# h33p/ofps

Measured on AMD Instinct MI355X. Metric: Mvectors/s, 1080p 16x16 blocks +-16 full-search SAD, higher is better.
Workload: dtype u8

## Files before the change

ofps_amd/csrc/sad.hip:

```cpp
#include "common.hpp"

#include <cstdlib>
#include <utility>

namespace {

constexpr int kWavesPerWG = 4;

constexpr int pick_stride(int min_s, int k, int ng) {
    for (int s = min_s; s < min_s + 64; ++s)
        if ((k * s) % 32 == ng % 32) return s;
    return min_s | 1;
}

template <int B, int R, int K>
struct SadCfg {
    static_assert(B % 4 == 0 && R % 4 == 0, "tile origin must stay dword aligned");
    static_assert(B * B * 255 <= 65535, "packed u16 SAD accumulators would overflow");
    static constexpr int NCAND = 2 * R + 1;
    static constexpr int NG = (NCAND + 3) / 4;
    static constexpr int NC = (NCAND + K - 1) / K;
    static constexpr int T = NG * NC;
    static constexpr int PASSES = (T + 63) / 64;
    static constexpr int BW = B / 4;
    static constexpr int TILE_H = B + 2 * R;
    static constexpr int TILE_ROWS = NC * K + B - 1;
    static constexpr int TILE_WD = (kWavesPerWG * B + 2 * R) / 4;
    static constexpr int MAXCOL = (kWavesPerWG - 1) * BW + (NG - 1) + BW;
    static constexpr int MIN_S = (MAXCOL + 1 > TILE_WD) ? MAXCOL + 1 : TILE_WD;
    static constexpr int S = pick_stride(MIN_S, K, NG);
    static constexpr int LDS_DWORDS = TILE_ROWS * S;
};

__device__ __forceinline__ unsigned long long shfl_xor_u64(unsigned long long v, int mask) {
    unsigned lo = (unsigned)v, hi = (unsigned)(v >> 32);
    lo = __shfl_xor(lo, mask, 64);
    hi = __shfl_xor(hi, mask, 64);
    return ((unsigned long long)hi << 32) | lo;
}

struct __attribute__((packed, aligned(4))) U64A4 { unsigned long long v; };

struct SadParams {
    const uint8_t* prev_base;
    const uint8_t* cur_base;
    size_t prev_pitch, cur_pitch;
    int W, H, stride;
    int nbx, nby;
    float nx, ny;
    float4* out_entries;
    int* out_best;
    unsigned long long div_spp, div_spr;
};
inline unsigned long long div_magic48(unsigned d) { return ((1ull << 48) + d - 1) / d; }
__device__ __forceinline__ unsigned div48(unsigned n, unsigned long long m) { return (unsigned)(((unsigned long long)n * m) >> 48); }

__device__ __forceinline__ void write_block_result(const SadParams& p, int pair, int bx, int by, int B, int R,
                                                   unsigned long long key) {
    const int sad = (int)(key >> 48);
    const int dy = (int)((key >> 8) & 0xFF) - R;
    const int dx = (int)(key & 0xFF) - R;
    const size_t k = ((size_t)pair * p.nby + by) * p.nbx + bx;
    const float cx = (float)(bx * B + B / 2 + dx), cy = (float)(by * B + B / 2 + dy);
    float4 e;
    e.x = cx * p.nx;
    e.y = cy * p.ny;
    e.z = ((float)dx / 1.0f) * (-p.nx);
    e.w = ((float)dy / 1.0f) * (-p.ny);
    p.out_entries[k] = e;
    if (p.out_best) {
        p.out_best[3 * k + 0] = dx;
        p.out_best[3 * k + 1] = dy;
        p.out_best[3 * k + 2] = sad;
    }
}

template <int B, int R, int K>
__global__ __launch_bounds__(256) void sad_qsad_kernel(const SadParams p) {
    using C = SadCfg<B, R, K>;
    __shared__ uint32_t tile[C::LDS_DWORDS];

    const int pair = blockIdx.z;
    const uint8_t* __restrict__ prev = p.prev_base + (size_t)pair * p.prev_pitch;
    const uint8_t* __restrict__ cur = p.cur_base + (size_t)pair * p.cur_pitch;
    const int by = blockIdx.y;
    const int bx0 = blockIdx.x * kWavesPerWG;
    const int tid = threadIdx.x;

    const int wave = __builtin_amdgcn_readfirstlane(tid >> 6);
    const int lane = tid & 63;
    const int bx = bx0 + wave;
    const int x0 = bx * B, y0 = by * B;

    uint32_t c[B][C::BW];
    {
        const int bxc = bx < p.nbx ? bx : p.nbx - 1;
        const uint32_t* __restrict__ cp = reinterpret_cast<const uint32_t*>(cur + (size_t)y0 * p.stride + bxc * B);
        const int sdw = p.stride >> 2;
#pragma unroll
        for (int y = 0; y < B; ++y)
#pragma unroll
            for (int q = 0; q < C::BW; ++q) c[y][q] = cp[y * sdw + q];
    }

    {
        const int tx0 = bx0 * B - R, ty0 = by * B - R;
        for (int idx = tid; idx < C::TILE_H * C::TILE_WD; idx += 256) {
            const int row = idx / C::TILE_WD, col = idx - row * C::TILE_WD;
            const int gx = tx0 + 4 * col, gy = ty0 + row;
            if (gy >= 0 && gy < p.H && gx >= 0 && gx < p.W)
                tile[row * C::S + col] = *reinterpret_cast<const uint32_t*>(prev + (size_t)gy * p.stride + gx);
        }
    }
    __syncthreads();
    if (bx >= p.nbx) return;

    unsigned long long best = ~0ull;
#pragma unroll 1
    for (int pass = 0; pass < C::PASSES; ++pass) {
        const int t = pass * 64 + lane;
        const bool active = t < C::T;
        const int tc = active ? t : 0;
        const int chunk = tc / C::NG, g = tc - chunk * C::NG;
        const int dx0 = -R + 4 * g, dy0 = -R + K * chunk;

        unsigned long long acc[K];
#pragma unroll
        for (int i = 0; i < K; ++i) acc[i] = 0;

        const uint32_t* trow = tile + (K * chunk) * C::S + wave * C::BW + g;
#pragma unroll
        for (int rr = 0; rr < B + K - 1; ++rr) {
            unsigned long long win[C::BW];
#pragma unroll
            for (int q = 0; q < C::BW; ++q) win[q] = reinterpret_cast<const U64A4*>(trow + rr * C::S + q)->v;
#pragma unroll
            for (int i = 0; i < K; ++i) {
                const int y = rr - i;
                if (y >= 0 && y < B) {
#pragma unroll
                    for (int q = 0; q < C::BW; ++q) acc[i] = __builtin_amdgcn_qsad_pk_u16_u8(win[q], c[y][q], acc[i]);
                }
            }
        }
        __builtin_amdgcn_sched_group_barrier(0x100, C::BW, 0);
#pragma unroll
        for (int rr = 0; rr < B + K - 1; ++rr) {
            __builtin_amdgcn_sched_group_barrier(0x100, C::BW, 0);
            __builtin_amdgcn_sched_group_barrier(0x002, K * C::BW, 0);
        }

#pragma unroll
        for (int i = 0; i < K; ++i) asm volatile("" : "+v"(acc[i]));

        uint32_t bkey = 0xFFFFFFFFu;
        int bci = 0;
#pragma unroll
        for (int i = 0; i < K; ++i) {
            const int dy = dy0 + i;
            const int vy = (int)active & (int)(dy <= R) & (int)(y0 + dy >= 0) & (int)(y0 + dy + B <= p.H);
#pragma unroll
            for (int j = 0; j < 4; ++j) {
                const int dx = dx0 + j;
                const int v = vy & (int)(dx <= R) & (int)(x0 + dx >= 0) & (int)(x0 + dx + B <= p.W);
                const uint32_t d2inv = (uint32_t)(dx * dx + dy * dy) | (uint32_t)(v - 1);
                const uint32_t half = (j < 2) ? (uint32_t)acc[i] : (uint32_t)(acc[i] >> 32);
                const uint32_t key = ((j & 1) ? (half & 0xFFFF0000u) : (half << 16)) | d2inv;
                const bool lt = key < bkey;
                bkey = lt ? key : bkey;
                bci = lt ? (i * 4 + j) : bci;
            }
        }
        if (bkey != 0xFFFFFFFFu) {
            const int bi = bci >> 2, bj = bci & 3;
            const unsigned long long k64 =
                ((unsigned long long)bkey << 32) | (uint32_t)(((dy0 + bi + R) << 8) | (dx0 + bj + R));
            best = k64 < best ? k64 : best;
        }
    }

#pragma unroll
    for (int m = 32; m >= 1; m >>= 1) {
        const unsigned long long o = shfl_xor_u64(best, m);
        best = o < best ? o : best;
    }
    if (lane == 0) write_block_result(p, pair, bx, by, B, R, best);
}

template <int B, int R>
struct StripCfg {
    static_assert(B % 4 == 0 && R % 4 == 0, "tile origin and the dx = +R column must stay dword aligned");
    static_assert(B * B * 255 <= 65535, "packed u16 SAD accumulators would overflow");
    static constexpr int NCAND = 2 * R + 1;
    static constexpr int NGA = (2 * R) / 4;
    static constexpr int pow2_ceil(int v) { int p = 1; while (p < v) p <<= 1; return p; }
    static constexpr int NG = pow2_ceil(NGA);
    static_assert(NGA >= 1 && NG <= 64, "search range too wide for one wave per strip");
    static constexpr int NB = 64 / NG;
    static constexpr int BW = B / 4;
    static constexpr int TILE_H = B + 2 * R;
    static constexpr int KE = (NCAND + NG - 1) / NG;
    static constexpr int EDGE_COL = (2 * R) / 4;
    static constexpr int GRAN = ((NB * B) % 16 == 0 && R % 16 == 0) ? 16 : (((NB * B) % 8 == 0 && R % 8 == 0) ? 8 : 4);
    static constexpr int GDW = GRAN / 4;
    static constexpr int TILE_WG = (NB * B + 2 * R + GRAN - 1) / GRAN;
    static constexpr int MAXCOL = (NB - 1) * BW + (NG - 1) + BW;
    static constexpr int SW = ((MAXCOL + 1 > TILE_WG * GDW ? MAXCOL + 1 : TILE_WG * GDW) + 3) / 4 * 4;
    static_assert((NB - 1) * BW + EDGE_COL + BW <= SW, "edge column must lie inside a window row");
    static constexpr int TILE_ROWS = TILE_H > NG * KE + B - 1 ? TILE_H : NG * KE + B - 1;
    static constexpr int TILE_DWORDS = TILE_ROWS * SW;
    static_assert(2 * R * R < 65536, "lane key holds d2 in 16 bits");
    static constexpr int SPLIT = (NCAND + 32) / 33;
    static constexpr int NP = (NCAND + SPLIT - 1) / SPLIT;
    static constexpr int MIN_WAVES = (2 * NP + B * BW + 40 <= 168) ? 3 : 2;
    static constexpr bool COMPACT_KEY = ((2 * R * R) << 6) + NCAND < 65536 && NCAND <= 64;
    static constexpr bool RANK_KEY = !COMPACT_KEY && ((2 * R * R) << 3) + 7 < 65536;
    static constexpr int KSHIFT = COMPACT_KEY ? 6 : (RANK_KEY ? 3 : 0);
};

template <int B, int R>
struct StripWalk {
    static constexpr int ROWS_PER_BASE = (255 - StripCfg<B, R>::BW) / StripCfg<B, R>::SW + 1;
};

template <int B, int R, int I0, int RR>
__device__ __forceinline__ void strip_row(unsigned long long (&acc)[StripCfg<B, R>::NP], const uint32_t (&c)[B][B / 4],
                                          const uint32_t* lds, uint32_t& base) {
    using C = StripCfg<B, R>;
    constexpr int G = StripWalk<B, R>::ROWS_PER_BASE;
    if constexpr (RR > 0 && RR % G == 0) {
        base += G * C::SW;
        asm volatile("" : "+v"(base));
    }
    unsigned long long win[C::BW];
#pragma unroll
    for (int q = 0; q < C::BW; ++q) win[q] = reinterpret_cast<const U64A4*>(lds + base + (RR % G) * C::SW + q)->v;
#pragma unroll
    for (int ii = 0; ii < C::NP; ++ii) {
        const int y = RR - ii;
        if (I0 + ii < C::NCAND && y >= 0 && y < B) {
#pragma unroll
            for (int q = 0; q < C::BW; ++q) acc[ii] = __builtin_amdgcn_qsad_pk_u16_u8(win[q], c[y][q], acc[ii]);
        }
    }
}

template <int B, int R, int I0, int... RR>
__device__ __forceinline__ void strip_rows(unsigned long long (&acc)[StripCfg<B, R>::NP], const uint32_t (&c)[B][B / 4],
                                           const uint32_t* lds, uint32_t tile_off, std::integer_sequence<int, RR...>) {
    uint32_t base = tile_off + I0 * StripCfg<B, R>::SW;
    asm volatile("" : "+v"(base));
    (strip_row<B, R, I0, RR>(acc, c, lds, base), ...);
}

#ifndef OFPS_SAD_COLKEYS
#define OFPS_SAD_COLKEYS 2
#endif
constexpr int kSadColKeys = OFPS_SAD_COLKEYS;
constexpr int kColSlotDwords = kSadColKeys == 2 ? 4 * 64 : 0;

template <int B, int R, int I0>
__device__ __forceinline__ void strip_pass(const uint32_t (&c)[B][B / 4], const uint32_t* lds, uint32_t tile_off,
                                           const uint32_t (&colk)[4], const uint32_t (&colk_pos)[4], int y0, int H, uint32_t& bkey, int& bi,
                                           uint32_t (&colmin)[4], uint32_t* amin) {
    using C = StripCfg<B, R>;
    unsigned long long acc[C::NP];
#pragma unroll
    for (int ii = 0; ii < C::NP; ++ii) acc[ii] = 0;
    constexpr int ROWS = ((I0 + C::NP < C::NCAND ? C::NP : C::NCAND - I0) + B - 1);
    strip_rows<B, R, I0>(acc, c, lds, tile_off, std::make_integer_sequence<int, ROWS>{});
#pragma unroll
    for (int ii = 0; ii < C::NP; ++ii) asm volatile("" : "+v"(acc[ii]));
    if constexpr (kSadColKeys != 0 && (C::RANK_KEY || C::COMPACT_KEY)) {
        auto low_of = [&](int ii) -> uint32_t {
            const int i = I0 + ii, dy = -R + i;
            const bool ok = i < C::NCAND && y0 + dy >= 0 && y0 + dy + B <= H;
            return ok ? (uint32_t)(C::RANK_KEY ? ((dy * dy) << 1 | (dy > 0 ? 1 : 0)) : ((dy * dy) << 6 | i)) : 0xFFFFFFFFu;
        };
        uint32_t hmask = 0xFFFF0000u;
        asm volatile("" : "+v"(hmask));
        auto keys_of = [&](int ii, uint32_t low, uint32_t (&k)[4]) {
            const uint32_t lo = (uint32_t)acc[ii], hi = (uint32_t)(acc[ii] >> 32);
            k[0] = (lo << 16) | low; k[1] = (lo & hmask) | low; k[2] = (hi << 16) | low; k[3] = (hi & hmask) | low;
        };
        if constexpr (kSadColKeys == 1) {
#pragma unroll
            for (int ii = 0; ii < C::NP; ii += 2) {
                if (I0 + ii >= C::NCAND) break;
                uint32_t ka[4], kb[4];
                keys_of(ii, low_of(ii), ka);
                if (ii + 1 < C::NP && I0 + ii + 1 < C::NCAND) {
                    keys_of(ii + 1, low_of(ii + 1), kb);
#pragma unroll
                    for (int j = 0; j < 4; ++j)
                        asm("v_min3_u32 %0, %1, %2, %3" : "=v"(colmin[j]) : "v"(colmin[j]), "v"(ka[j]), "v"(kb[j]));
                } else {
#pragma unroll
                    for (int j = 0; j < 4; ++j) colmin[j] = min(colmin[j], ka[j]);
                }
            }
        } else {
#pragma unroll
            for (int ii = 0; ii < C::NP; ++ii) {
                if (I0 + ii >= C::NCAND) break;
                uint32_t k[4];
                keys_of(ii, low_of(ii), k);
#pragma unroll
                for (int j = 0; j < 4; ++j) __hip_atomic_fetch_min(amin + 64 * j, k[j], __ATOMIC_RELAXED, __HIP_MEMORY_SCOPE_WAVEFRONT);
            }
        }
        return;
    }
#pragma unroll
    for (int ii = 0; ii < C::NP; ++ii) {
        const int i = I0 + ii;
        const int dy = -R + i;
        if (i < C::NCAND && y0 + dy >= 0 && y0 + dy + B <= H) {
            const uint32_t lo = (uint32_t)acc[ii], hi = (uint32_t)(acc[ii] >> 32);
            const uint32_t (&ck)[4] = (C::RANK_KEY && dy > 0) ? colk_pos : colk;
            const uint32_t k0 = (lo << 16) | ck[0];
            const uint32_t k1 = (lo & 0xFFFF0000u) | ck[1];
            const uint32_t k2 = (hi << 16) | ck[2];
            const uint32_t k3 = (hi & 0xFFFF0000u) | ck[3];
            if constexpr (C::RANK_KEY) {
                bkey = min(bkey, __builtin_elementwise_add_sat(min(min(k0, k1), min(k2, k3)), (uint32_t)((dy * dy) << 3)));
            } else if constexpr (C::COMPACT_KEY) {
                const uint32_t m = __builtin_elementwise_add_sat(min(min(k0, k1), min(k2, k3)), (uint32_t)((dy * dy) << 6 | i));
                bkey = min(bkey, m);
            } else {
                const uint32_t m = __builtin_elementwise_add_sat(min(min(k0, k1), min(k2, k3)), (uint32_t)(dy * dy));
                const bool lt = m < bkey;
                bkey = lt ? m : bkey;
                bi = lt ? i : bi;
            }
        }
    }
}

template <int B, int R, int... S>
__device__ __forceinline__ void strip_passes(const uint32_t (&c)[B][B / 4], const uint32_t* lds, uint32_t tile_off,
                                             const uint32_t (&colk)[4], const uint32_t (&colk_pos)[4], int y0, int H, uint32_t& bkey, int& bi,
                                             uint32_t (&colmin)[4], uint32_t* amin, std::integer_sequence<int, S...>) {
    (strip_pass<B, R, S * StripCfg<B, R>::NP>(c, lds, tile_off, colk, colk_pos, y0, H, bkey, bi, colmin, amin), ...);
}

constexpr int kStripWaves = 4;

template <int B, int R>
__device__ __forceinline__ void strip_body(const SadParams& p, int strips_per_row, int strip, uint32_t* tiles, int wave, int lane) {
    using C = StripCfg<B, R>;
    const int strips_per_pair = strips_per_row * p.nby;
    const int pair = (int)div48((unsigned)strip, p.div_spp);
    const int rem = strip - pair * strips_per_pair;
    const int by = (int)div48((unsigned)rem, p.div_spr);
    const int bx0 = (rem - by * strips_per_row) * C::NB;

    const uint8_t* __restrict__ prev = p.prev_base + (size_t)pair * p.prev_pitch;
    const uint8_t* __restrict__ cur = p.cur_base + (size_t)pair * p.cur_pitch;
    uint32_t* tile = tiles + wave * C::TILE_DWORDS;

    const int b = lane / C::NG;
    const int g = lane % C::NG;
    const int bx = bx0 + b;
    const bool blk_on = bx < p.nbx;
    const int y0 = by * B;

    uint32_t c[B][C::BW];
    {
        const int bxc = blk_on ? bx : p.nbx - 1;
        const uint8_t* cp = cur + (size_t)y0 * p.stride + bxc * B;
#pragma unroll
        for (int y = 0; y < B; ++y) {
            if constexpr (C::BW % 4 == 0) {
#pragma unroll
                for (int q4 = 0; q4 < C::BW; q4 += 4) {
                    const uint4 v = *reinterpret_cast<const uint4*>(cp + (size_t)y * p.stride + 4 * q4);
                    c[y][q4 + 0] = v.x; c[y][q4 + 1] = v.y; c[y][q4 + 2] = v.z; c[y][q4 + 3] = v.w;
                }
            } else {
#pragma unroll
                for (int q2 = 0; q2 < C::BW; q2 += 2) {
                    const uint2 v = *reinterpret_cast<const uint2*>(cp + (size_t)y * p.stride + 4 * q2);
                    c[y][q2 + 0] = v.x; c[y][q2 + 1] = v.y;
                }
            }
        }
    }

    {
        constexpr int LR = 64 / C::TILE_WG;
        constexpr int STEPS = (C::TILE_H + LR - 1) / LR;
        const int tx0 = bx0 * B - R, ty0 = y0 - R;
        const int sr = lane / C::TILE_WG, sc = lane - sr * C::TILE_WG;
        const int gx = tx0 + C::GRAN * sc;
        const bool lane_on = sr < LR && gx >= 0 && gx < p.W;
        const uint8_t* src = prev + (ptrdiff_t)(ty0 + sr) * p.stride + gx;
        uint32_t* dst = tile + sr * C::SW + C::GDW * sc;
#pragma unroll
        for (int it = 0; it < STEPS; ++it) {
            const int row = sr + it * LR;
            const bool row_in_tile = (it + 1) * LR <= C::TILE_H || row < C::TILE_H;
            if (lane_on && row_in_tile && (unsigned)(ty0 + row) < (unsigned)p.H) {
                const uint8_t* sp = src + (ptrdiff_t)(it * LR) * p.stride;
                uint32_t* dp = dst + it * LR * C::SW;
                if constexpr (C::GRAN == 16) *reinterpret_cast<uint4*>(dp) = *reinterpret_cast<const uint4*>(sp);
                else if constexpr (C::GRAN == 8) *reinterpret_cast<uint2*>(dp) = *reinterpret_cast<const uint2*>(sp);
                else *dp = *reinterpret_cast<const uint32_t*>(sp);
            }
        }
    }
    __builtin_amdgcn_fence(__ATOMIC_RELEASE, "wavefront");
    __builtin_amdgcn_wave_barrier();
    __builtin_amdgcn_fence(__ATOMIC_ACQUIRE, "wavefront");

    const int dx0 = -R + 4 * g;
    uint32_t colk[4], colk_pos[4];
#pragma unroll
    for (int j = 0; j < 4; ++j) {
        const int dx = dx0 + j;
        const int x = bx * B + dx;
        const bool v = blk_on && g < C::NGA && x >= 0 && x + B <= p.W;
        const uint32_t rank = dx0 < 0 ? 3u - j : (uint32_t)j;
        colk[j] = v ? ((uint32_t)(dx * dx) << C::KSHIFT) | (C::RANK_KEY ? rank : 0u) : 0xFFFFFFFFu;
        colk_pos[j] = v ? ((uint32_t)(dx * dx) << C::KSHIFT) | (7u - rank) : 0xFFFFFFFFu;
    }
    uint32_t bkey = 0xFFFFFFFFu;
    int bi = 0;
    uint32_t colmin[4] = {0xFFFFFFFFu, 0xFFFFFFFFu, 0xFFFFFFFFu, 0xFFFFFFFFu};
    uint32_t* amin = nullptr;
    if constexpr (kSadColKeys == 2 && (C::RANK_KEY || C::COMPACT_KEY)) {
        amin = tiles + kStripWaves * C::TILE_DWORDS + wave * kColSlotDwords + lane;
#pragma unroll
        for (int j = 0; j < 4; ++j) amin[64 * j] = 0xFFFFFFFFu;
    }
    strip_passes<B, R>(c, tiles, (uint32_t)(wave * C::TILE_DWORDS + b * C::BW + g), colk, colk_pos, y0, p.H, bkey, bi, colmin, amin,
                       std::make_integer_sequence<int, C::SPLIT>{});
    if constexpr (kSadColKeys != 0 && (C::RANK_KEY || C::COMPACT_KEY)) {
#pragma unroll
        for (int j = 0; j < 4; ++j) {
            uint32_t kc;
            if constexpr (kSadColKeys == 2) kc = __hip_atomic_load(amin + 64 * j, __ATOMIC_RELAXED, __HIP_MEMORY_SCOPE_WAVEFRONT);
            else kc = colmin[j];
            uint32_t lk;
            if constexpr (C::RANK_KEY) {
                const uint32_t x = (((kc & 0xFFFEu) << 2) + colk[j]) ^ ((kc & 1u) * 7u);
                lk = (kc & 0xFFFF0000u) | x;
            } else {
                lk = (kc & 0xFFFF0000u) | ((kc & 0xFFFFu) + colk[j]);
            }
            lk = (colk[j] == 0xFFFFFFFFu || kc == 0xFFFFFFFFu) ? 0xFFFFFFFFu : lk;
            bkey = min(bkey, lk);
        }
    }
    unsigned long long best = ~0ull;
    if (bkey != 0xFFFFFFFFu) {
        const uint32_t d2 = (bkey & 0xFFFFu) >> C::KSHIFT;
        int dx = dx0, dy;
        if constexpr (C::RANK_KEY) {
            const int code = (int)(bkey & 7u);
            const bool neg = code < 4;
            const int rank = neg ? code : 7 - code;
            dx = dx0 + (dx0 < 0 ? 3 - rank : rank);
            const int ady = (int)(__builtin_sqrtf((float)((int)d2 - dx * dx)) + 0.5f);
            dy = neg ? -ady : ady;
        } else {
            if constexpr (C::COMPACT_KEY) bi = (int)(bkey & 63u);
            dy = -R + bi;
            const int dxsq = (int)d2 - dy * dy;
#pragma unroll
            for (int j = 1; j < 4; ++j) dx = ((dx0 + j) * (dx0 + j) == dxsq) ? dx0 + j : dx;
        }
        best = ((unsigned long long)((bkey & 0xFFFF0000u) | d2) << 32) | (unsigned long long)(uint32_t)(((dy + R) << 8) | (dx + R));
    }
    uint32_t eacc[C::KE];
#pragma unroll
    for (int i = 0; i < C::KE; ++i) eacc[i] = 0;
    {
        const uint32_t* ecol = tile + b * C::BW + C::EDGE_COL;
        const int erow0 = g * C::KE;
        uint32_t nxt[C::BW];
#pragma unroll
        for (int q = 0; q < C::BW; ++q) nxt[q] = ecol[erow0 * C::SW + q];
#pragma unroll
        for (int rr = 0; rr < B + C::KE - 1; ++rr) {
            uint32_t ref[C::BW];
#pragma unroll
            for (int q = 0; q < C::BW; ++q) ref[q] = nxt[q];
            if (rr + 1 < B + C::KE - 1) {
                const int row = erow0 + rr + 1;
#pragma unroll
                for (int q = 0; q < C::BW; ++q) nxt[q] = ecol[row * C::SW + q];
            }
#pragma unroll
            for (int i = 0; i < C::KE; ++i) {
                const int y = rr - i;
                if (y >= 0 && y < B) {
#pragma unroll
                    for (int q = 0; q < C::BW; ++q) eacc[i] = __builtin_amdgcn_sad_u8(ref[q], c[y][q], eacc[i]);
                }
            }
            asm volatile("" : "+v"(eacc[0]) : : "memory");
        }
    }

    {
        const bool xok = blk_on && bx * B + R + B <= p.W;
#pragma unroll
        for (int i = 0; i < C::KE; ++i) {
            const int dy = -R + g * C::KE + i;
            const bool v = xok && dy <= R && y0 + dy >= 0 && y0 + dy + B <= p.H;
            const unsigned long long k64 =
                ((unsigned long long)((eacc[i] << 16) | (uint32_t)(R * R + dy * dy)) << 32) |
                (unsigned long long)(uint32_t)(((dy + R) << 8) | (2 * R));
            best = (v && k64 < best) ? k64 : best;
        }
    }
#pragma unroll
    for (int m = 1; m < C::NG; m <<= 1) {
        const unsigned long long o = shfl_xor_u64(best, m);
        best = o < best ? o : best;
    }
    if (blk_on && g == 0) {
        const int sad = (int)(best >> 48);
        const int dy = (int)((best >> 8) & 0xFF) - R, dx = (int)(best & 0xFF) - R;
        const size_t k = ((size_t)pair * p.nby + by) * p.nbx + bx;
        float4 e;
        e.x = (float)(bx * B + B / 2 + dx) * p.nx;
        e.y = (float)(y0 + B / 2 + dy) * p.ny;
        e.z = ((float)dx / 1.0f) * (-p.nx);
        e.w = ((float)dy / 1.0f) * (-p.ny);
        p.out_entries[k] = e;
        if (p.out_best) {
            p.out_best[3 * k + 0] = dx;
            p.out_best[3 * k + 1] = dy;
            p.out_best[3 * k + 2] = sad;
        }
    }
}

template <int B, int R>
__global__ __launch_bounds__(64 * kStripWaves, (StripCfg<B, R>::MIN_WAVES)) void sad_strip_kernel(const SadParams p, int strips_per_row,
                                                                      int total_strips) {
    using C = StripCfg<B, R>;
    __shared__ __attribute__((aligned(16))) uint32_t tiles[kStripWaves * (C::TILE_DWORDS + kColSlotDwords)];
    const int wave = __builtin_amdgcn_readfirstlane(threadIdx.x >> 6);
    const int lane = threadIdx.x & 63;
    const int per_xcd = gridDim.x / 8;
    const int lwg = (int)(blockIdx.x % 8) * per_xcd + (int)(blockIdx.x / 8);
    const int strip = lwg * kStripWaves + wave;
    if (strip >= total_strips) return;
    strip_body<B, R>(p, strips_per_row, strip, tiles, wave, lane);
}

template <int B, int R>
__global__ __launch_bounds__(64 * kStripWaves, (StripCfg<B, R>::MIN_WAVES)) void sad_strip_list_kernel(const SadParams p, int strips_per_row,
                                                                           const uint32_t* __restrict__ strip_list) {
    using C = StripCfg<B, R>;
    __shared__ __attribute__((aligned(16))) uint32_t tiles[kStripWaves * (C::TILE_DWORDS + kColSlotDwords)];
    const int wave = __builtin_amdgcn_readfirstlane(threadIdx.x >> 6);
    const int lane = threadIdx.x & 63;
    const int count = (int)strip_list[0];
#pragma unroll 1
    for (int k = (int)blockIdx.x * kStripWaves + wave; k < count; k += (int)gridDim.x * kStripWaves)
        strip_body<B, R>(p, strips_per_row, (int)strip_list[1 + k], tiles, wave, lane);
}

struct PdeCfg {
    static constexpr int B = 16, R = 16, STEP = 4, PR = B / STEP;
    using C = StripCfg<B, R>;
    static constexpr int CUR_DW = B * C::NB * C::BW;
    static constexpr int CAP = 512;
    static constexpr int WAVE_DW = C::TILE_DWORDS + 4 + CUR_DW + CAP + 2 * C::NB;
    static constexpr int OFF_CUR = C::TILE_DWORDS + 4, OFF_LIST = OFF_CUR + CUR_DW, OFF_BEST = OFF_LIST + CAP;
    static_assert(OFF_BEST % 2 == 0, "64-bit keys must be 8-byte aligned");
};

template <int RR>
__device__ __forceinline__ void pde_row(unsigned long long (&acc)[PdeCfg::C::NP], const uint32_t (&c)[PdeCfg::PR][PdeCfg::C::BW],
                                        const uint32_t* lds, uint32_t& base) {
    using C = PdeCfg::C;
    constexpr int B = PdeCfg::B, R = PdeCfg::R, STEP = PdeCfg::STEP;
    constexpr int G = StripWalk<B, R>::ROWS_PER_BASE;
    if constexpr (RR > 0 && RR % G == 0) {
        base += G * C::SW;
        asm volatile("" : "+v"(base));
    }
    unsigned long long win[C::BW];
#pragma unroll
    for (int q = 0; q < C::BW; ++q) win[q] = reinterpret_cast<const U64A4*>(lds + base + (RR % G) * C::SW + q)->v;
#pragma unroll
    for (int ii = 0; ii < C::NP; ++ii) {
        const int y = RR - ii;
        if (ii < C::NCAND && y >= 0 && y < B && y % STEP == 0) {
#pragma unroll
            for (int q = 0; q < C::BW; ++q) acc[ii] = __builtin_amdgcn_qsad_pk_u16_u8(win[q], c[y / STEP][q], acc[ii]);
        }
    }
}
template <int... RR>
__device__ __forceinline__ void pde_rows(unsigned long long (&acc)[PdeCfg::C::NP], const uint32_t (&c)[PdeCfg::PR][PdeCfg::C::BW],
                                         const uint32_t* lds, uint32_t tile_off, std::integer_sequence<int, RR...>) {
    uint32_t base = tile_off;
    asm volatile("" : "+v"(base));
    (pde_row<RR>(acc, c, lds, base), ...);
}

__device__ __forceinline__ uint32_t pde_two_rows(const uint32_t* tile, const uint32_t* curl, int bb, int dyi, int dxi, int r8) {
    using C = PdeCfg::C;
    const int sh = dxi & 3;
    uint32_t s = 0;
#pragma unroll
    for (int k = 0; k < 2; ++k) {
        const int y = 2 * r8 + k;
        const uint32_t* rp = tile + (dyi + y) * C::SW + bb * C::BW + (dxi >> 2);
        const uint32_t* cp = curl + y * (C::NB * C::BW) + bb * C::BW;
        uint32_t d[C::BW + 1];
#pragma unroll
        for (int q = 0; q <= C::BW; ++q) d[q] = rp[q];
#pragma unroll
        for (int q = 0; q < C::BW; ++q) s = __builtin_amdgcn_sad_u8(__builtin_amdgcn_alignbyte(d[q + 1], d[q], sh), cp[q], s);
    }
    return s;
}

__global__ __launch_bounds__(64 * kStripWaves, 3) void sad_pde_kernel(const SadParams p, int strips_per_row, int total_strips,
                                                                       uint32_t* __restrict__ strip_list) {
    using P = PdeCfg;
    using C = P::C;
    constexpr int B = P::B, R = P::R;
    __shared__ __attribute__((aligned(16))) uint32_t lds[kStripWaves * P::WAVE_DW];

    const int wave = __builtin_amdgcn_readfirstlane(threadIdx.x >> 6);
    const int lane = threadIdx.x & 63;
    const int per_xcd = gridDim.x / 8;
    const int lwg = (int)(blockIdx.x % 8) * per_xcd + (int)(blockIdx.x / 8);
    const int strip = lwg * kStripWaves + wave;
    if (strip >= total_strips) return;
    const int strips_per_pair = strips_per_row * p.nby;
    const int pair = strip / strips_per_pair;
    const int rem = strip - pair * strips_per_pair;
    const int by = rem / strips_per_row;
    const int bx0 = (rem - by * strips_per_row) * C::NB;
    const uint8_t* __restrict__ prev = p.prev_base + (size_t)pair * p.prev_pitch;
    const uint8_t* __restrict__ cur = p.cur_base + (size_t)pair * p.cur_pitch;
    uint32_t* tile = lds + wave * P::WAVE_DW;
    uint32_t* curl = tile + P::OFF_CUR;
    uint32_t* list = tile + P::OFF_LIST;
    unsigned long long* bestk = reinterpret_cast<unsigned long long*>(tile + P::OFF_BEST);

    const int b = lane / C::NG, g = lane % C::NG;
    const int bx = bx0 + b;
    const bool blk_on = bx < p.nbx;
    const int y0 = by * B;

    {
        const int tx0 = bx0 * B - R, ty0 = y0 - R;
        for (int idx = lane; idx < C::TILE_H * C::TILE_WG; idx += 64) {
            const int row = idx / C::TILE_WG, col = idx - row * C::TILE_WG;
            const int gx = tx0 + 16 * col, gy = ty0 + row;
            if (gy >= 0 && gy < p.H && gx >= 0 && gx < p.W)
                *reinterpret_cast<uint4*>(tile + row * C::SW + 4 * col) = *reinterpret_cast<const uint4*>(prev + (size_t)gy * p.stride + gx);
        }
#pragma unroll
        for (int k = 0; k < 2; ++k) {
            const int idx = lane + 64 * k, row = idx / C::NB, blk = idx % C::NB;
            const int bxc = min(bx0 + blk, p.nbx - 1);
            *reinterpret_cast<uint4*>(curl + row * (C::NB * C::BW) + blk * C::BW) =
                *reinterpret_cast<const uint4*>(cur + (size_t)(y0 + row) * p.stride + bxc * B);
        }
    }
    __builtin_amdgcn_fence(__ATOMIC_RELEASE, "wavefront");
    __builtin_amdgcn_wave_barrier();
    __builtin_amdgcn_fence(__ATOMIC_ACQUIRE, "wavefront");

    uint32_t c4[P::PR][C::BW];
#pragma unroll
    for (int r = 0; r < P::PR; ++r)
#pragma unroll
        for (int q = 0; q < C::BW; ++q) c4[r][q] = curl[(P::STEP * r) * (C::NB * C::BW) + b * C::BW + q];
    unsigned long long acc[C::NP];
#pragma unroll
    for (int ii = 0; ii < C::NP; ++ii) acc[ii] = 0;
    pde_rows(acc, c4, lds, (uint32_t)(wave * P::WAVE_DW + b * C::BW + g), std::make_integer_sequence<int, C::NCAND + B - 1>{});
#pragma unroll
    for (int ii = 0; ii < C::NP; ++ii) asm volatile("" : "+v"(acc[ii]));

    const int dx0 = -R + 4 * g;
    bool colv[4];
    uint32_t colk[4];
#pragma unroll
    for (int j = 0; j < 4; ++j) {
        const int x = bx * B + dx0 + j;
        colv[j] = blk_on && x >= 0 && x + B <= p.W;
        colk[j] = colv[j] ? (uint32_t)((dx0 + j) * (dx0 + j)) << C::KSHIFT : 0xFFFFFFFFu;
    }
    static_assert(C::COMPACT_KEY && C::SPLIT == 1, "written for the +-16 geometry");
    uint32_t bkey = 0xFFFFFFFFu;
#pragma unroll
    for (int i = 0; i < C::NCAND; ++i) {
        const int dy = -R + i;
        if (y0 + dy >= 0 && y0 + dy + B <= p.H) {
            const uint32_t lo = (uint32_t)acc[i], hi = (uint32_t)(acc[i] >> 32);
            const uint32_t k0 = (lo << 16) | colk[0], k1 = (lo & 0xFFFF0000u) | colk[1];
            const uint32_t k2 = (hi << 16) | colk[2], k3 = (hi & 0xFFFF0000u) | colk[3];
            bkey = min(bkey, __builtin_elementwise_add_sat(min(min(k0, k1), min(k2, k3)), (uint32_t)((dy * dy) << 6 | i)));
        }
    }
    unsigned long long pbest = ~0ull;
    if (bkey != 0xFFFFFFFFu) {
        const int bi = (int)(bkey & 63u), dy = -R + bi;
        const uint32_t d2 = (bkey & 0xFFFFu) >> C::KSHIFT;
        const int dxsq = (int)d2 - dy * dy;
        int dx = dx0;
#pragma unroll
        for (int j = 1; j < 4; ++j) dx = ((dx0 + j) * (dx0 + j) == dxsq) ? dx0 + j : dx;
        pbest = ((unsigned long long)((bkey & 0xFFFF0000u) | d2) << 32) | (unsigned long long)(uint32_t)(((dy + R) << 8) | (dx + R));
    }
    uint32_t eacc[C::KE];
    const bool xok = blk_on && bx * B + R + B <= p.W;
    {
        const uint32_t* ecol = tile + b * C::BW + C::EDGE_COL;
#pragma unroll
        for (int i = 0; i < C::KE; ++i) {
            const int dyi = min(g * C::KE + i, C::NCAND - 1);
            uint32_t sacc = 0;
#pragma unroll
            for (int r = 0; r < P::PR; ++r)
#pragma unroll
                for (int q = 0; q < C::BW; ++q) sacc = __builtin_amdgcn_sad_u8(ecol[(dyi + P::STEP * r) * C::SW + q], c4[r][q], sacc);
            eacc[i] = sacc;
            const int dy = -R + g * C::KE + i;
            const bool v = xok && dy <= R && y0 + dy >= 0 && y0 + dy + B <= p.H;
            const unsigned long long k64 = ((unsigned long long)((sacc << 16) | (uint32_t)(R * R + dy * dy)) << 32) |
                                           (unsigned long long)(uint32_t)(((dy + R) << 8) | (2 * R));
            pbest = (v && k64 < pbest) ? k64 : pbest;
        }
    }
#pragma unroll
    for (int m = 1; m < C::NG; m <<= 1) {
        const unsigned long long o = shfl_xor_u64(pbest, m);
        pbest = o < pbest ? o : pbest;
    }
    const int dy0i = blk_on ? (int)((pbest >> 8) & 0xFF) : R, dx0i = blk_on ? (int)(pbest & 0xFF) : R;
    auto key64 = [&](uint32_t sad, int dyi, int dxi) {
        const int dy = dyi - R, dx = dxi - R;
        return ((unsigned long long)((sad << 16) | (uint32_t)(dx * dx + dy * dy)) << 32) | (unsigned long long)(uint32_t)((dyi << 8) | dxi);
    };
    uint32_t U = pde_two_rows(tile, curl, b, dy0i, dx0i, g);
#pragma unroll
    for (int m = 1; m < C::NG; m <<= 1) U += __shfl_xor(U, m, 64);
    if (g == 0) bestk[b] = blk_on ? key64(U, dy0i, dx0i) : ~0ull;
    int nlist = 0;
    {
        int uj[4];
#pragma unroll
        for (int j = 0; j < 4; ++j) uj[j] = colv[j] ? (int)U : -1;
        const unsigned long long below = (1ull << lane) - 1ull;
        typedef unsigned short us2 __attribute__((ext_vector_type(2)));
        const uint32_t u1 = min(U + 1u, 0xFFFFu) * 0x10001u;
        auto any_le = [&](uint32_t v) {
            const us2 m = __builtin_elementwise_min(__builtin_bit_cast(us2, v), __builtin_bit_cast(us2, u1));
            return __builtin_bit_cast(uint32_t, m) ^ u1;
        };
#pragma unroll
        for (int i = 0; i < C::NCAND; ++i) {
            const int dy = -R + i;
            if (y0 + dy >= 0 && y0 + dy + B <= p.H) {
                const uint32_t lo = (uint32_t)acc[i], hi = (uint32_t)(acc[i] >> 32);
                if (!__ballot((any_le(lo) | any_le(hi)) != 0u)) continue;
                const int s4[4] = {(int)(lo & 0xFFFFu), (int)(lo >> 16), (int)(hi & 0xFFFFu), (int)(hi >> 16)};
#pragma unroll
                for (int j = 0; j < 4; ++j) {
                    const bool hit = s4[j] <= uj[j];
                    const unsigned long long mask = __ballot(hit);
                    if (mask) {
                        const int pos = nlist + __popcll(mask & below);
                        if (hit && pos < P::CAP) list[pos] = ((uint32_t)b << 16) | ((uint32_t)i << 8) | (uint32_t)(4 * g + j);
                        nlist += __popcll(mask);
                    }
                }
            }
        }
#pragma unroll
        for (int i = 0; i < C::KE; ++i) {
            const int dyi = g * C::KE + i, dy = dyi - R;
            const bool hit = xok && dy <= R && y0 + dy >= 0 && y0 + dy + B <= p.H && eacc[i] <= U;
            const unsigned long long mask = __ballot(hit);
            if (mask) {
                const int pos = nlist + __popcll(mask & below);
                if (hit && pos < P::CAP) list[pos] = ((uint32_t)b << 16) | ((uint32_t)dyi << 8) | (uint32_t)(2 * R);
                nlist += __popcll(mask);
            }
        }
    }
    __builtin_amdgcn_fence(__ATOMIC_RELEASE, "wavefront");
    __builtin_amdgcn_wave_barrier();
    __builtin_amdgcn_fence(__ATOMIC_ACQUIRE, "wavefront");
    const int n = nlist;
    if (n > P::CAP) {
        if (lane == 0) {
            const uint32_t pos = atomicAdd(&strip_list[0], 1u);
            strip_list[1 + pos] = (uint32_t)strip;
        }
        return;
    }
    constexpr int PER_STEP = 2 * (64 / C::NG);
    for (int base = 0; base < n; base += PER_STEP) {
        const int idx0 = base + lane / C::NG, idx1 = idx0 + 64 / C::NG;
        const uint32_t e0 = list[min(idx0, n - 1)], e1 = list[min(idx1, n - 1)];
        const int bb0 = (int)(e0 >> 16), dyi0 = (int)((e0 >> 8) & 0xFF), dxi0 = (int)(e0 & 0xFF);
        const int bb1 = (int)(e1 >> 16), dyi1 = (int)((e1 >> 8) & 0xFF), dxi1 = (int)(e1 & 0xFF);
        uint32_t s0 = pde_two_rows(tile, curl, bb0, dyi0, dxi0, g);
        uint32_t s1 = pde_two_rows(tile, curl, bb1, dyi1, dxi1, g);
#pragma unroll
        for (int m = 1; m < C::NG; m <<= 1) { s0 += __shfl_xor(s0, m, 64); s1 += __shfl_xor(s1, m, 64); }
        if (g == 0 && idx0 < n) atomicMin(&bestk[bb0], key64(s0, dyi0, dxi0));
        if (g == 0 && idx1 < n) atomicMin(&bestk[bb1], key64(s1, dyi1, dxi1));
    }
    __builtin_amdgcn_fence(__ATOMIC_RELEASE, "wavefront");
    __builtin_amdgcn_wave_barrier();
    __builtin_amdgcn_fence(__ATOMIC_ACQUIRE, "wavefront");
    if (blk_on && g == 0) write_block_result(p, pair, bx, by, B, R, bestk[b]);
}

__global__ __launch_bounds__(64) void sad_generic_kernel(const SadParams p, int B, int R) {
    const int pair = blockIdx.z, by = blockIdx.y, bx = blockIdx.x;
    const uint8_t* __restrict__ prev = p.prev_base + (size_t)pair * p.prev_pitch;
    const uint8_t* __restrict__ cur = p.cur_base + (size_t)pair * p.cur_pitch;
    const int x0 = bx * B, y0 = by * B, n = 2 * R + 1;
    unsigned long long best = ~0ull;
    for (int cand = threadIdx.x; cand < n * n; cand += 64) {
        const int dy = cand / n - R, dx = cand % n - R;
        if (x0 + dx < 0 || x0 + dx + B > p.W || y0 + dy < 0 || y0 + dy + B > p.H) continue;
        uint32_t sad = 0;
        for (int y = 0; y < B; ++y) {
            const uint8_t* cr = cur + (size_t)(y0 + y) * p.stride + x0;
            const uint8_t* pr = prev + (size_t)(y0 + dy + y) * p.stride + x0 + dx;
            for (int x = 0; x < B; ++x) {
                const int d = (int)cr[x] - (int)pr[x];
                sad += (uint32_t)(d < 0 ? -d : d);
            }
        }
        const unsigned long long key = ((unsigned long long)sad << 32) | ((unsigned long long)(dx * dx + dy * dy) << 16) |
                                       (unsigned long long)(((dy + R) << 8) | (dx + R));
        best = key < best ? key : best;
    }
#pragma unroll
    for (int m = 32; m >= 1; m >>= 1) {
        const unsigned long long o = shfl_xor_u64(best, m);
        best = o < best ? o : best;
    }
    if (threadIdx.x == 0) {
        const int sad = (int)(best >> 32);
        const int dy = (int)((best >> 8) & 0xFF) - R, dx = (int)(best & 0xFF) - R;
        const size_t k = ((size_t)pair * p.nby + by) * p.nbx + bx;
        float4 e;
        e.x = (float)(x0 + B / 2 + dx) * p.nx;
        e.y = (float)(y0 + B / 2 + dy) * p.ny;
        e.z = ((float)dx / 1.0f) * (-p.nx);
        e.w = ((float)dy / 1.0f) * (-p.ny);
        p.out_entries[k] = e;
        if (p.out_best) {
            p.out_best[3 * k + 0] = dx;
            p.out_best[3 * k + 1] = dy;
            p.out_best[3 * k + 2] = sad;
        }
    }
}

template <int B, int R, int K>
void launch_qsad(const SadParams& p, int pairs, hipStream_t s) {
    dim3 grid((p.nbx + kWavesPerWG - 1) / kWavesPerWG, p.nby, pairs);
    hipLaunchKernelGGL((sad_qsad_kernel<B, R, K>), grid, dim3(256), 0, s, p);
}

inline void strip_div_magic(SadParams& q, int strips_per_row) {
    q.div_spp = div_magic48((unsigned)strips_per_row * (unsigned)q.nby);
    q.div_spr = div_magic48((unsigned)strips_per_row);
}

template <int B, int R>
void launch_strip(const SadParams& p, int pairs, hipStream_t s) {
    using C = StripCfg<B, R>;
    const int strips_per_row = (p.nbx + C::NB - 1) / C::NB;
    const int total = strips_per_row * p.nby * pairs;
    const int nwg = ((total + kStripWaves - 1) / kStripWaves + 7) / 8 * 8;
    SadParams q = p;
    strip_div_magic(q, strips_per_row);
    hipLaunchKernelGGL((sad_strip_kernel<B, R>), dim3(nwg), dim3(64 * kStripWaves), 0, s, q, strips_per_row, total);
}

int launch_pde_16_16(ofps_hip_ctx* ctx, const SadParams& p, int pairs, hipStream_t s) {
    using C = StripCfg<16, 16>;
    const int strips_per_row = (p.nbx + C::NB - 1) / C::NB;
    const int total = strips_per_row * p.nby * pairs;
    auto* strip_list = static_cast<uint32_t*>(ofps::scratch(ctx, ofps::S_SAD_LIST, (size_t)(total + 1) * sizeof(uint32_t)));
    if (!strip_list) return OFPS_HIP_ENOMEM;
    OFPS_HIP_TRY(ctx, hipMemsetAsync(strip_list, 0, sizeof(uint32_t), s));
    const int nwg = ((total + kStripWaves - 1) / kStripWaves + 7) / 8 * 8;
    hipLaunchKernelGGL(sad_pde_kernel, dim3(nwg), dim3(64 * kStripWaves), 0, s, p, strips_per_row, total, strip_list);
    const int nwg_ind = nwg < 8 * ctx->num_cus ? nwg : 8 * ctx->num_cus;
    SadParams q = p;
    strip_div_magic(q, strips_per_row);
    hipLaunchKernelGGL((sad_strip_list_kernel<16, 16>), dim3(nwg_ind), dim3(64 * kStripWaves), 0, s, q, strips_per_row,
                       (const uint32_t*)strip_list);
    return OFPS_HIP_OK;
}

}

extern "C" {

size_t ofps_hip_sad_block_count(int W, int H, int block) {
    if (W <= 0 || H <= 0 || block <= 0) return 0;
    return (size_t)(W / block) * (size_t)(H / block);
}

}

namespace ofps {
int sad_pairs_device(ofps_hip_ctx* ctx, const uint8_t* prev_base, size_t prev_pitch, const uint8_t* cur_base,
                     size_t cur_pitch, int pairs, int W, int H, int stride, int block, int range, void* d_out_entries,
                     void* d_out_best, bool integer_only, void* d_int_best) {
    OFPS_REQUIRE(ctx, W > 0 && H > 0 && stride >= W, "sad_flow: bad geometry W=%d H=%d stride=%d", W, H, stride);
    OFPS_REQUIRE(ctx, stride % 4 == 0 && ((uintptr_t)prev_base % 4) == 0 && ((uintptr_t)cur_base % 4) == 0 &&
                          prev_pitch % 4 == 0 && cur_pitch % 4 == 0,
                 "sad_flow: rows must be 4-byte aligned (stride=%d)", stride);
    OFPS_REQUIRE(ctx, block >= 1 && block <= 64 && range >= 0 && range <= 64,
                 "sad_flow: block=%d range=%d outside [1,64]/[0,64]", block, range);
    SadParams p{};
    p.prev_base = prev_base; p.cur_base = cur_base;
    p.prev_pitch = prev_pitch; p.cur_pitch = cur_pitch;
    p.W = W; p.H = H; p.stride = stride;
    p.nbx = W / block; p.nby = H / block;
    p.nx = 1.0f / (float)W; p.ny = 1.0f / (float)H;
    p.out_entries = static_cast<float4*>(d_out_entries);
    p.out_best = static_cast<int*>(d_out_best);
    if (p.nbx == 0 || p.nby == 0 || pairs <= 0) return OFPS_HIP_OK;
    OFPS_REQUIRE(ctx, pairs <= 65535 && p.nby <= 65535, "sad_flow: grid too large");
    OFPS_HIP_TRY(ctx, hipSetDevice(ctx->device));
    const bool qpel = ctx->opt.sad_motion_scale == 4 && !integer_only;
    if (qpel && d_int_best) p.out_best = static_cast<int*>(d_int_best);
    else if (qpel && !p.out_best) {
        p.out_best = static_cast<int*>(ofps::scratch(ctx, ofps::S_SAD_QBEST, (size_t)pairs * p.nbx * p.nby * 3 * sizeof(int)));
        if (!p.out_best) return OFPS_HIP_ENOMEM;
    }
    hipStream_t s = ctx->stream;
    const int key = block * 1000 + range;
    const bool force_block = ctx->opt.sad_force_block != 0;
    const bool strip_ok = !force_block && stride % 16 == 0 && ((uintptr_t)prev_base % 16) == 0 &&
                          ((uintptr_t)cur_base % 16) == 0 && prev_pitch % 16 == 0 && cur_pitch % 16 == 0 &&
                          (long long)p.nbx * p.nby * pairs < (1ll << 28) && (long long)p.nbx * p.nby < (1ll << 20);
    switch (key) {
        case 16016:
            if (strip_ok && ctx->sad_mode == OFPS_HIP_SAD_PRUNED) {
                const int rc = launch_pde_16_16(ctx, p, pairs, s);
                if (rc != OFPS_HIP_OK) return rc;
            } else if (strip_ok) launch_strip<16, 16>(p, pairs, s);
            else launch_qsad<16, 16, 5>(p, pairs, s);
            break;
        case 16008:
            if (strip_ok) launch_strip<16, 8>(p, pairs, s); else launch_qsad<16, 8, 3>(p, pairs, s);
            break;
        case 16032:
            if (strip_ok) launch_strip<16, 32>(p, pairs, s); else launch_qsad<16, 32, 5>(p, pairs, s);
            break;
        case 8032:
            if (strip_ok) launch_strip<8, 32>(p, pairs, s); else launch_qsad<8, 32, 5>(p, pairs, s);
            break;
        case 8016:
            if (strip_ok) launch_strip<8, 16>(p, pairs, s); else launch_qsad<8, 16, 5>(p, pairs, s);
            break;
        case 8008:
            if (strip_ok) launch_strip<8, 8>(p, pairs, s); else launch_qsad<8, 8, 3>(p, pairs, s);
            break;
#define OFPS_STRIP_CASE(BB, RR)                                         \
        case BB * 1000 + RR:                                            \
            if (strip_ok) { launch_strip<BB, RR>(p, pairs, s); break; } \
            [[fallthrough]];
        OFPS_STRIP_CASE(16, 12) OFPS_STRIP_CASE(16, 20) OFPS_STRIP_CASE(16, 24) OFPS_STRIP_CASE(16, 28)
        OFPS_STRIP_CASE(8, 12) OFPS_STRIP_CASE(8, 20) OFPS_STRIP_CASE(8, 24) OFPS_STRIP_CASE(8, 28)
#undef OFPS_STRIP_CASE
        default: {
            dim3 grid(p.nbx, p.nby, pairs);
            hipLaunchKernelGGL(sad_generic_kernel, grid, dim3(64), 0, s, p, block, range);
        }
    }
    OFPS_HIP_TRY(ctx, hipGetLastError());
    if (qpel)
        return ofps::sad_qpel_refine_device(ctx, prev_base, prev_pitch, cur_base, cur_pitch, pairs, W, H, stride, block, range, d_out_entries,
                                            p.out_best, d_out_best);
    return OFPS_HIP_OK;
}
}

extern "C" {

int ofps_hip_sad_flow_dev(ofps_hip_ctx* ctx, const void* d_frames, int n_frames, int W, int H, int stride,
                          size_t frame_pitch, int ref_mode, int block, int range, void* d_out_entries,
                          void* d_out_best) {
    if (!ctx) return OFPS_HIP_EINVAL;
    OFPS_REQUIRE(ctx, d_frames && d_out_entries, "sad_flow: null device pointer");
    OFPS_REQUIRE(ctx, n_frames >= 2, "sad_flow: need at least 2 frames (got %d)", n_frames);
    OFPS_REQUIRE(ctx, frame_pitch >= (size_t)stride * (size_t)H, "sad_flow: frame_pitch smaller than a frame");
    OFPS_REQUIRE(ctx, ref_mode == 0 || ref_mode == 1, "sad_flow: ref_mode must be 0 or 1");
    const auto* f = static_cast<const uint8_t*>(d_frames);
    return ofps::sad_pairs_device(ctx, f, ref_mode ? 0 : frame_pitch, f + frame_pitch, frame_pitch, n_frames - 1, W, H, stride,
                                  block, range, d_out_entries, d_out_best);
}

int ofps_hip_sad_flow(ofps_hip_ctx* ctx, const uint8_t* prev, const uint8_t* cur, int W, int H, int stride,
                      int block, int range, float* out_entries, int32_t* out_best, size_t* n_out) {
    if (!ctx) return OFPS_HIP_EINVAL;
    OFPS_REQUIRE(ctx, prev && cur && out_entries, "sad_flow: null host pointer");
    OFPS_REQUIRE(ctx, W > 0 && H > 0 && stride >= W && block >= 1, "sad_flow: bad geometry");
    OFPS_HIP_TRY(ctx, hipSetDevice(ctx->device));
    const int dstride = (W + 63) & ~63;
    const size_t pitch = (size_t)dstride * H;
    const size_t nblk = ofps_hip_sad_block_count(W, H, block);
    auto* d_frames = static_cast<uint8_t*>(ofps::scratch(ctx, ofps::S_FRAMES, 2 * pitch));
    auto* d_ent = static_cast<float*>(ofps::scratch(ctx, ofps::S_ENTRIES, nblk * 4 * sizeof(float)));
    auto* d_best = static_cast<int32_t*>(ofps::scratch(ctx, ofps::S_BEST, nblk * 3 * sizeof(int32_t)));
    if (!d_frames || !d_ent || !d_best) return OFPS_HIP_ENOMEM;
    OFPS_HIP_TRY(ctx, ofps::upload_rows(d_frames, dstride, prev, stride, W, H, ctx->stream));
    OFPS_HIP_TRY(ctx, ofps::upload_rows(d_frames + pitch, dstride, cur, stride, W, H, ctx->stream));
    if (ctx->opt.sad_gate > 0 || ctx->opt.sad_consistency > 0) {
        auto* d_kept = static_cast<uint32_t*>(ofps::scratch(ctx, ofps::S_RESULT, sizeof(uint32_t)));
        if (!d_kept) return OFPS_HIP_ENOMEM;
        int rc = ctx->opt.sad_consistency > 0
                     ? ofps::sad_flow_checked_device(ctx, d_frames, d_frames + pitch, W, H, dstride, block, range, ctx->opt.sad_gate,
                                                     ctx->opt.sad_consistency, reinterpret_cast<float4*>(d_ent), out_best ? d_best : nullptr, d_kept)
                     : ofps::sad_flow_gated_device(ctx, d_frames, d_frames + pitch, W, H, dstride, block, range, ctx->opt.sad_gate,
                                                   reinterpret_cast<float4*>(d_ent), out_best ? d_best : nullptr, d_kept);
        if (rc != OFPS_HIP_OK) return rc;
        uint32_t kept = 0;
        OFPS_HIP_TRY(ctx, hipMemcpyAsync(&kept, d_kept, sizeof(kept), hipMemcpyDeviceToHost, ctx->stream));
        if (nblk) {
            OFPS_HIP_TRY(ctx, hipMemcpyAsync(out_entries, d_ent, nblk * 4 * sizeof(float), hipMemcpyDeviceToHost, ctx->stream));
            if (out_best)
                OFPS_HIP_TRY(ctx, hipMemcpyAsync(out_best, d_best, nblk * 3 * sizeof(int32_t), hipMemcpyDeviceToHost, ctx->stream));
        }
        OFPS_HIP_TRY(ctx, hipStreamSynchronize(ctx->stream));
        if (n_out) *n_out = kept < nblk ? kept : nblk;
        return OFPS_HIP_OK;
    }
    int rc = ofps_hip_sad_flow_dev(ctx, d_frames, 2, W, H, dstride, pitch, 0, block, range, d_ent, d_best);
    if (rc != OFPS_HIP_OK) return rc;
    if (nblk) {
        OFPS_HIP_TRY(ctx, hipMemcpyAsync(out_entries, d_ent, nblk * 4 * sizeof(float), hipMemcpyDeviceToHost, ctx->stream));
        if (out_best)
            OFPS_HIP_TRY(ctx, hipMemcpyAsync(out_best, d_best, nblk * 3 * sizeof(int32_t), hipMemcpyDeviceToHost, ctx->stream));
    }
    OFPS_HIP_TRY(ctx, hipStreamSynchronize(ctx->stream));
    if (n_out) *n_out = nblk;
    return OFPS_HIP_OK;
}

int ofps_hip_sad_pruned_overflow_strips(ofps_hip_ctx* ctx, uint32_t* count) {
    if (!ctx || !count) return OFPS_HIP_EINVAL;
    *count = 0;
    auto& sc = ctx->scratch[ofps::S_SAD_LIST];
    if (!sc.p) return OFPS_HIP_OK;
    OFPS_HIP_TRY(ctx, hipSetDevice(ctx->device));
    OFPS_HIP_TRY(ctx, hipStreamSynchronize(ctx->stream));
    OFPS_HIP_TRY(ctx, hipMemcpy(count, sc.p, sizeof(uint32_t), hipMemcpyDeviceToHost));
    return OFPS_HIP_OK;
}

int ofps_hip_set_sad_mode(ofps_hip_ctx* ctx, int mode) {
    if (!ctx) return OFPS_HIP_EINVAL;
    OFPS_REQUIRE(ctx, mode == OFPS_HIP_SAD_EXHAUSTIVE || mode == OFPS_HIP_SAD_PRUNED, "set_sad_mode: unknown mode %d", mode);
    ctx->sad_mode = mode;
    return OFPS_HIP_OK;
}

}
```

Before: 519.5.

## Add clipped-row strip path, scalar-base loads, and DPP row-shift min reduction

Adds a separate loop for strips at the top and bottom image edges that evaluates only the valid dy candidates, so out-of-frame rows are not computed. Current-frame and tile loads now use a scalar base pointer plus a 32-bit offset, aiming to cut 64-bit VGPR address arithmetic. The xor-shuffle min reduction is replaced with DPP row_shl moves, and low keys are hinted into SGPRs. Risks: the DPP row_shl reduction leaves the full minimum only in lane g==0 of each group, which must line up with group boundaries; the clipped path is a rolled loop that could be slower per candidate; and the strip wave count becomes a macro.

After: 519.6 (median of 2 runs). About the same (+0.0%).

```diff
diff --git a/ofps_amd/csrc/sad.hip b/ofps_amd/csrc/sad.hip
--- a/ofps_amd/csrc/sad.hip
+++ b/ofps_amd/csrc/sad.hip
@@ -37,6 +37,26 @@
     lo = __shfl_xor(lo, mask, 64);
     hi = __shfl_xor(hi, mask, 64);
     return ((unsigned long long)hi << 32) | lo;
+}
+
+template <int M>
+__device__ __forceinline__ unsigned long long min_row_shl(unsigned long long v) {
+    const int lo = (int)(unsigned)v, hi = (int)(unsigned)(v >> 32);
+    const unsigned olo = (unsigned)__builtin_amdgcn_mov_dpp(lo, 0x100 + M, 0xF, 0xF, true);
+    const unsigned ohi = (unsigned)__builtin_amdgcn_mov_dpp(hi, 0x100 + M, 0xF, 0xF, true);
+    const unsigned long long o = ((unsigned long long)ohi << 32) | olo;
+    return o < v ? o : v;
+}
+
+template <class T>
+__device__ __forceinline__ T load_sbase(const uint8_t* sbase, uint32_t off) {
+#if defined(__HIP_DEVICE_COMPILE__)
+    asm("" : "+s"(sbase));
+    typedef const __attribute__((address_space(1))) uint8_t* gptr;
+    return *reinterpret_cast<const __attribute__((address_space(1))) T*>((gptr)sbase + off);
+#else
+    return *reinterpret_cast<const T*>(sbase + off);
+#endif
 }
 
 struct __attribute__((packed, aligned(4))) U64A4 { unsigned long long v; };
@@ -275,7 +295,9 @@
         auto low_of = [&](int ii) -> uint32_t {
             const int i = I0 + ii, dy = -R + i;
             const bool ok = i < C::NCAND && y0 + dy >= 0 && y0 + dy + B <= H;
-            return ok ? (uint32_t)(C::RANK_KEY ? ((dy * dy) << 1 | (dy > 0 ? 1 : 0)) : ((dy * dy) << 6 | i)) : 0xFFFFFFFFu;
+            uint32_t low = ok ? (uint32_t)(C::RANK_KEY ? ((dy * dy) << 1 | (dy > 0 ? 1 : 0)) : ((dy * dy) << 6 | i)) : 0xFFFFFFFFu;
+            asm("" : "+s"(low));
+            return low;
         };
         uint32_t hmask = 0xFFFF0000u;
         asm volatile("" : "+v"(hmask));
@@ -344,7 +366,41 @@
     (strip_pass<B, R, S * StripCfg<B, R>::NP>(c, lds, tile_off, colk, colk_pos, y0, H, bkey, bi, colmin, amin), ...);
 }
 
-constexpr int kStripWaves = 4;
+template <int B, int R>
+__device__ __forceinline__ void strip_pass_clipped(const uint32_t (&c)[B][B / 4], const uint32_t* lds, uint32_t tile_off, int y0, int H,
+                                                   uint32_t (&colmin)[4], uint32_t* amin) {
+    using C = StripCfg<B, R>;
+    const int i_lo = y0 < R ? R - y0 : 0;
+    const int i_hi = H - B - y0 < R ? H - B - y0 + R : 2 * R;
+    uint32_t hmask = 0xFFFF0000u;
+    asm volatile("; ofps_clip_begin" : "+v"(hmask));
+#pragma unroll 1
+    for (int i = i_lo; i <= i_hi; ++i) {
+        const uint32_t base = tile_off + (uint32_t)i * C::SW;
+        unsigned long long acc = 0;
+#pragma unroll
+        for (int y = 0; y < B; ++y) {
+#pragma unroll
+            for (int q = 0; q < C::BW; ++q)
+                acc = __builtin_amdgcn_qsad_pk_u16_u8(reinterpret_cast<const U64A4*>(lds + base + y * C::SW + q)->v, c[y][q], acc);
+        }
+        const int dy = i - R;
+        const uint32_t low = C::RANK_KEY ? (uint32_t)((dy * dy) << 1 | (dy > 0 ? 1 : 0)) : (uint32_t)((dy * dy) << 6 | i);
+        const uint32_t lo = (uint32_t)acc, hi = (uint32_t)(acc >> 32);
+        const uint32_t k[4] = {(lo << 16) | low, (lo & hmask) | low, (hi << 16) | low, (hi & hmask) | low};
+#pragma unroll
+        for (int j = 0; j < 4; ++j) {
+            if constexpr (kSadColKeys == 2) __hip_atomic_fetch_min(amin + 64 * j, k[j], __ATOMIC_RELAXED, __HIP_MEMORY_SCOPE_WAVEFRONT);
+            else colmin[j] = min(colmin[j], k[j]);
+        }
+    }
+    asm volatile("; ofps_clip_end" : "+v"(hmask));
+}
+
+#ifndef OFPS_SAD_STRIP_WAVES
+#define OFPS_SAD_STRIP_WAVES 4
+#endif
+constexpr int kStripWaves = OFPS_SAD_STRIP_WAVES;
 
 template <int B, int R>
 __device__ __forceinline__ void strip_body(const SadParams& p, int strips_per_row, int strip, uint32_t* tiles, int wave, int lane) {
@@ -368,19 +424,21 @@
     uint32_t c[B][C::BW];
     {
         const int bxc = blk_on ? bx : p.nbx - 1;
-        const uint8_t* cp = cur + (size_t)y0 * p.stride + bxc * B;
+        const uint32_t coff = (uint32_t)(bxc * B);
+        const uint8_t* crow = cur + (size_t)y0 * p.stride;
 #pragma unroll
         for (int y = 0; y < B; ++y) {
+            const uint8_t* cp = crow + (size_t)y * p.stride;
             if constexpr (C::BW % 4 == 0) {
 #pragma unroll
                 for (int q4 = 0; q4 < C::BW; q4 += 4) {
-                    const uint4 v = *reinterpret_cast<const uint4*>(cp + (size_t)y * p.stride + 4 * q4);
+                    const uint4 v = load_sbase<uint4>(cp, coff + 4 * q4);
                     c[y][q4 + 0] = v.x; c[y][q4 + 1] = v.y; c[y][q4 + 2] = v.z; c[y][q4 + 3] = v.w;
                 }
             } else {
 #pragma unroll
                 for (int q2 = 0; q2 < C::BW; q2 += 2) {
-                    const uint2 v = *reinterpret_cast<const uint2*>(cp + (size_t)y * p.stride + 4 * q2);
+                    const uint2 v = load_sbase<uint2>(cp, coff + 4 * q2);
                     c[y][q2 + 0] = v.x; c[y][q2 + 1] = v.y;
                 }
             }
@@ -394,18 +452,19 @@
         const int sr = lane / C::TILE_WG, sc = lane - sr * C::TILE_WG;
         const int gx = tx0 + C::GRAN * sc;
         const bool lane_on = sr < LR && gx >= 0 && gx < p.W;
-        const uint8_t* src = prev + (ptrdiff_t)(ty0 + sr) * p.stride + gx;
+        const uint8_t* worg = prev + (ptrdiff_t)ty0 * p.stride + tx0;
+        const uint32_t soff = (uint32_t)(sr * p.stride + C::GRAN * sc);
         uint32_t* dst = tile + sr * C::SW + C::GDW * sc;
 #pragma unroll
         for (int it = 0; it < STEPS; ++it) {
             const int row = sr + it * LR;
             const bool row_in_tile = (it + 1) * LR <= C::TILE_H || row < C::TILE_H;
             if (lane_on && row_in_tile && (unsigned)(ty0 + row) < (unsigned)p.H) {
-                const uint8_t* sp = src + (ptrdiff_t)(it * LR) * p.stride;
+                const uint8_t* srow = worg + (ptrdiff_t)(it * LR) * p.stride;
                 uint32_t* dp = dst + it * LR * C::SW;
-                if constexpr (C::GRAN == 16) *reinterpret_cast<uint4*>(dp) = *reinterpret_cast<const uint4*>(sp);
-                else if constexpr (C::GRAN == 8) *reinterpret_cast<uint2*>(dp) = *reinterpret_cast<const uint2*>(sp);
-                else *dp = *reinterpret_cast<const uint32_t*>(sp);
+                if constexpr (C::GRAN == 16) *reinterpret_cast<uint4*>(dp) = load_sbase<uint4>(srow, soff);
+                else if constexpr (C::GRAN == 8) *reinterpret_cast<uint2*>(dp) = load_sbase<uint2>(srow, soff);
+                else *dp = load_sbase<uint32_t>(srow, soff);
             }
         }
     }
@@ -433,8 +492,11 @@
 #pragma unroll
         for (int j = 0; j < 4; ++j) amin[64 * j] = 0xFFFFFFFFu;
     }
-    strip_passes<B, R>(c, tiles, (uint32_t)(wave * C::TILE_DWORDS + b * C::BW + g), colk, colk_pos, y0, p.H, bkey, bi, colmin, amin,
-                       std::make_integer_sequence<int, C::SPLIT>{});
+    const uint32_t tile_off = (uint32_t)(wave * C::TILE_DWORDS + b * C::BW + g);
+    if (kSadColKeys != 0 && (C::RANK_KEY || C::COMPACT_KEY) && (y0 < R || y0 + B + R > p.H))
+        strip_pass_clipped<B, R>(c, tiles, tile_off, y0, p.H, colmin, amin);
+    else
+        strip_passes<B, R>(c, tiles, tile_off, colk, colk_pos, y0, p.H, bkey, bi, colmin, amin, std::make_integer_sequence<int, C::SPLIT>{});
     if constexpr (kSadColKeys != 0 && (C::RANK_KEY || C::COMPACT_KEY)) {
 #pragma unroll
         for (int j = 0; j < 4; ++j) {
@@ -505,21 +567,23 @@
 
     {
         const bool xok = blk_on && bx * B + R + B <= p.W;
+        const int dy_lo = y0 < R ? -y0 : -R, dy_hi = p.H - B - y0 < R ? p.H - B - y0 : R;
+        const int dyg = -R + g * C::KE;
 #pragma unroll
         for (int i = 0; i < C::KE; ++i) {
-            const int dy = -R + g * C::KE + i;
-            const bool v = xok && dy <= R && y0 + dy >= 0 && y0 + dy + B <= p.H;
+            const int dy = dyg + i;
+            const bool v = xok && dyg >= dy_lo - i && dyg <= dy_hi - i;
             const unsigned long long k64 =
-                ((unsigned long long)((eacc[i] << 16) | (uint32_t)(R * R + dy * dy)) << 32) |
+                ((unsigned long long)((eacc[i] << 16) | (uint32_t)(R * R + __mul24(dy, dy))) << 32) |
                 (unsigned long long)(uint32_t)(((dy + R) << 8) | (2 * R));
             best = (v && k64 < best) ? k64 : best;
         }
     }
-#pragma unroll
-    for (int m = 1; m < C::NG; m <<= 1) {
-        const unsigned long long o = shfl_xor_u64(best, m);
-        best = o < best ? o : best;
-    }
+    static_assert(C::NG <= 16, "the reduction stays inside one DPP row");
+    if constexpr (C::NG > 1) best = min_row_shl<1>(best);
+    if constexpr (C::NG > 2) best = min_row_shl<2>(best);
+    if constexpr (C::NG > 4) best = min_row_shl<4>(best);
+    if constexpr (C::NG > 8) best = min_row_shl<8>(best);
     if (blk_on && g == 0) {
         const int sad = (int)(best >> 48);
         const int dy = (int)((best >> 8) & 0xFF) - R, dx = (int)(best & 0xFF) - R;
```
